# crowdbotp/socialways

Measured on AMD Instinct MI355X. Metric: GAN train steps/sec (256 scenes x 8 agents x 8+12 T per GPU step; fp32; social block on), higher is better.
Workload: dtype f32; 1 GPU; m1: 256 scenes x 8 agents x (8 obs + 12 pred) per GPU step = reference --batch-size 2048; use_social=True, n_unrolling_steps=1, info loss on; full=False, global_batch_scenes=256, parallelism=dp1, steps_per_graph_launch=32, settle_steps=992, rehearsal_regions=2, step_alg_bytes=5527040, inputs=z drawn on the host every step

## Files before the change

### socialways_amd/csrc/sw_wgrad.h

```cpp
#pragma once
#include <hip/hip_runtime.h>
#include <stddef.h>

#define SW_WG_MAXP 24
#define SW_WG_MAXSPLIT 256
#define SW_WG_WS_FLOATS ((size_t)SW_WG_MAXSPLIT * 65536)

struct WgProblem {
  const float* delta;
  const float* act;
  float* dW;
  float* db;
  float* db2;
  size_t ws_off;
  int ldd, lda, ldw, R, N, K, ones, accumulate;
  int nbn, nbk, nsplit, job0, out0;
  int pre;
  const float* act2;
  float* dW2;
  int lda2, ldw2, K2, row0;
};
struct WgBatch {
  int job0s[SW_WG_MAXP], out0s[SW_WG_MAXP];
  WgProblem p[SW_WG_MAXP];
  int np = 0, total_jobs = 0, total_out = 0;
  size_t top_reserved = 0;
};

struct WgAdam {
  float* w = nullptr;
  float* m = nullptr;
  float* v = nullptr;
  const float* g0 = nullptr;
  const float* step = nullptr;
  double lr = 0, beta1 = 0, beta2 = 0, eps = 0;
  size_t n = ~(size_t)0;
  const float* bc = nullptr;
  float* img = nullptr;
  const int* tab = nullptr;
};
__device__ __forceinline__ void wg_adam_bc_compute(const float* step, double beta1, double beta2, float& bc1, float& bc2s) {
  const float st = *step;
  bc1 = (float)(1 - pow(beta1, (double)st));
  bc2s = (float)sqrt(1 - pow(beta2, (double)st));
}
__device__ __forceinline__ void wg_adam_bc(const WgAdam& A, float& bc1, float& bc2s) {
  if (A.bc) {
    bc1 = A.bc[0];
    bc2s = A.bc[1];
    return;
  }
  wg_adam_bc_compute(A.step, A.beta1, A.beta2, bc1, bc2s);
}
struct WgAdamPre {
  size_t i;
  float m, v, w;
  int2 t;
};
__device__ __forceinline__ WgAdamPre wg_adam_pre(const WgAdam& A, const float* gptr) {
  WgAdamPre s;
  s.i = (size_t)(gptr - A.g0);
  s.t = int2{-1, -1};
  if (s.i >= A.n) {
    s.i = ~(size_t)0;
    s.m = s.v = s.w = 0.f;
    return s;
  }
  s.m = A.m[s.i];
  s.v = A.v[s.i];
  s.w = A.w[s.i];
  if (A.img) s.t = reinterpret_cast<const int2*>(A.tab)[s.i];
  return s;
}
__device__ __forceinline__ void wg_adam_fin(const WgAdam& A, const WgAdamPre& s, float bc1, float bc2s, float grad) {
  if (s.i == ~(size_t)0) return;
  const float m = (float)((double)s.m + (1 - A.beta1) * ((double)grad - (double)s.m));
  const float v = (float)(A.beta2 * s.v + (1 - A.beta2) * grad * grad);
  const float step_size = (float)(A.lr / bc1);
  const float denom = (float)((sqrtf(v) / bc2s) + A.eps);
  A.m[s.i] = m;
  A.v[s.i] = v;
  const float wn = s.w - step_size * m / denom;
  A.w[s.i] = wn;
  if (A.img) {
    if (s.t.x >= 0) A.img[s.t.x] = wn;
    if (s.t.y >= 0) A.img[s.t.y] = wn;
  }
}
__device__ __forceinline__ void wg_adam1(const WgAdam& A, float bc1, float bc2s, const float* gptr, float grad) {
  wg_adam_fin(A, wg_adam_pre(A, gptr), bc1, bc2s, grad);
}
int wg_reduce_launch_adam(WgBatch& b, float* ws, const WgAdam& ad, hipStream_t stream);
int wg_reduce_launch(WgBatch& b, float* ws, hipStream_t stream);
int wg_launch_adam(WgBatch& b, float* ws, WgAdam& ad, hipStream_t stream);

bool wg_shape_ok(int N, int K);
int wg_add(WgBatch& b, const float* delta, int ldd, const float* act, int lda, int R, int N, int K, float* dW,
           int ldw, float* db, float* db2, int accumulate);
int wg_add_tail(WgBatch& b, const float* delta, int ldd, const float* act, int lda, int R, int N, int K, float* dW,
                int ldw, const float* act2, int lda2, int K2, float* dW2, int ldw2, int row0, float* db, float* db2,
                int accumulate);
double wg_total_work(const WgBatch& b);
size_t wg_finalize(WgBatch& b);
int wg_launch(WgBatch& b, float* ws, hipStream_t stream);
int wg_add_pre(WgBatch& b, int N, int K, float* dW, int ldw, float* db, int nslices);
int wg_launch_finalized(WgBatch& b, float* ws, hipStream_t stream);
struct sw_wgrad_batch;
WgBatch* wg_pending(sw_wgrad_batch* h);
```

### socialways_amd/csrc/sw_wgrad.hip

```cpp
#include "../../include/socialways_hip.h"
#include "sw_common.h"
#include "sw_wgrad.h"
#include "sw_wgrad_dev.h"
#include <stdlib.h>

__host__ __device__ inline int wg_grid_jobs(int total_jobs) { return (total_jobs + 31) & ~31; }
#ifdef SW_WG_STAMP
__device__ unsigned long long g_wg_stamps[4 * 4096];
extern "C" int sw_debug_wg_stamps(unsigned long long* host, int n) {
  return hipMemcpyFromSymbol(host, HIP_SYMBOL(g_wg_stamps), sizeof(unsigned long long) * (size_t)n) == hipSuccess ? 0 : -1;
}
#endif
__global__ __launch_bounds__(SW_THREADS, 2) void wgrad_partial_kernel(WgBatch batch, float* __restrict__ ws,
                                                                      const float* __restrict__ adam_step, double beta1,
                                                                      double beta2, float* __restrict__ bc_out) {
  __shared__ __attribute__((aligned(16))) float red[SW_WG_RED_FLOATS];
  if ((int)blockIdx.x >= wg_grid_jobs(batch.total_jobs)) {
    if (threadIdx.x == 0) {
      float bc1, bc2s;
      wg_adam_bc_compute(adam_step, beta1, beta2, bc1, bc2s);
      bc_out[0] = bc1;
      bc_out[1] = bc2s;
    }
    return;
  }
  const int v = blockIdx.x, l = v >> 3;
  const int job = ((((l >> 2) << 3) + (v & 7)) << 2) + (l & 3);
  if (job >= batch.total_jobs) return;
#ifdef SW_WG_STAMP
  const unsigned long long t0 = wall_clock64();
#endif
  wg_job(batch, ws, job, red);
#ifdef SW_WG_STAMP
  if (threadIdx.x == 0 && blockIdx.x < 2048) {
    int p = 0;
    while (p + 1 < batch.np && job >= batch.job0s[p + 1]) ++p;
    unsigned long long* o = g_wg_stamps + (batch.total_jobs < 400 ? 4 * 2048 : 0) + 4 * blockIdx.x;
    o[0] = t0;
    o[1] = wall_clock64();
    o[2] = p;
    o[3] = batch.total_jobs;
  }
#endif
}
__device__ float g_wg_bc[2 * 64];
static float* wg_bc_slot() {
  static float* base[32] = {};
  static unsigned next = 0;
  int dev = -1;
  if (hipGetDevice(&dev) != hipSuccess || dev < 0 || dev >= 32) return nullptr;
  if (!base[dev]) {
    void* p = nullptr;
    if (hipGetSymbolAddress(&p, HIP_SYMBOL(g_wg_bc)) != hipSuccess) {
      (void)hipGetLastError();
      return nullptr;
    }
    base[dev] = (float*)p;
  }
  return base[dev] + 2 * (next++ % 64);
}

#ifndef SW_WG_RSUB
#define SW_WG_RSUB 4
#endif
#define SW_WG_REL (64 / SW_WG_RSUB)
__global__ __launch_bounds__(256) void wgrad_reduce_kernel(WgBatch batch, const float* __restrict__ ws, WgAdam ad) {
  const int gid = blockIdx.x * 256 + threadIdx.x;
  const int lane = gid & 63, el = lane % SW_WG_REL, sub = lane / SW_WG_REL;
  const int i = (gid >> 6) * SW_WG_REL + el;
  bool live = i < batch.total_out;
  int ii = live ? i : batch.total_out - 1;
  int p = 0;
#pragma unroll 1
  while (p + 1 < batch.np && ii >= batch.out0s[p + 1]) ++p;
  const WgProblem& P = batch.p[p];
  const int e = ii - P.out0;
  const int Kc = P.K + P.K2 + P.ones;
  const size_t stride = (size_t)P.N * Kc;
  const float* src = ws + P.ws_off + e;
  const int n = e / Kc, k = e - n * Kc;
  float* dst = k < P.K ? P.dW + (size_t)n * P.ldw + k : k < P.K + P.K2 ? P.dW2 + (size_t)n * P.ldw2 + (k - P.K) : P.db + n;
  float* dst2 = (k >= P.K + P.K2 && P.db2) ? P.db2 + n : nullptr;
  WgAdamPre a1 = {}, a2 = {};
  float old1 = 0.f, old2 = 0.f;
  if (ad.w) {
    a1 = wg_adam_pre(ad, dst);
    if (dst2) a2 = wg_adam_pre(ad, dst2);
  }
  if (P.accumulate) {
    old1 = *dst;
    if (dst2) old2 = *dst2;
  }
  float s = 0.f;
  float s1 = 0.f, s2 = 0.f, s3 = 0.f;
  int q = sub;
  for (; q + 3 * SW_WG_RSUB < P.nsplit; q += 4 * SW_WG_RSUB) {
    s += src[(size_t)q * stride];
    s1 += src[(size_t)(q + SW_WG_RSUB) * stride];
    s2 += src[(size_t)(q + 2 * SW_WG_RSUB) * stride];
    s3 += src[(size_t)(q + 3 * SW_WG_RSUB) * stride];
  }
  for (; q < P.nsplit; q += SW_WG_RSUB) s += src[(size_t)q * stride];
  s = (s + s1) + (s2 + s3);
#pragma unroll
  for (int o = SW_WG_REL; o < 64; o <<= 1) s += __shfl_xor(s, o);
  float bc1 = 1.f, bc2s = 1.f;
  if (ad.w) wg_adam_bc(ad, bc1, bc2s);
  if (!live || sub != 0) return;
  const float g = P.accumulate ? old1 + s : s;
  *dst = g;
  if (ad.w) wg_adam_fin(ad, a1, bc1, bc2s, g);
  if (dst2) {
    const float g2 = P.accumulate ? old2 + s : s;
    *dst2 = g2;
    if (ad.w) wg_adam_fin(ad, a2, bc1, bc2s, g2);
  }
}

bool wg_shape_ok(int N, int K) {
  for (int n0 = 0; n0 < N; n0 += 64)
    if (!wg_tiles(N - n0 < 64 ? N - n0 : 64, false)) return false;
  return K == 0 || wg_tiles(K, true) != 0;
}

static bool wg_span_ok(int R, int ld, int row0) {
  const long long rows = (long long)R / 4 + 4 + 8 * 4 * SW_WG_DEPTH + row0;
  return rows * ld * 4 < (1LL << 31);
}

int wg_add(WgBatch& b, const float* delta, int ldd, const float* act, int lda, int R, int N, int K, float* dW,
           int ldw, float* db, float* db2, int accumulate) {
  if (N > 256 || (ldd & 3) || (lda & 3)) return SW_ESHAPE;
  if (!wg_span_ok(R, ldd, 0) || !wg_span_ok(R, lda, 0)) return SW_ESHAPE;
  if (K < 1) return SW_ESHAPE;
  const int Nfull = N > 64 && (N & 63) && (N & 63) <= 32 && b.np + 2 * ((K + 63) / 64) <= SW_WG_MAXP ? (N & ~63) : N;
  for (int n0 = 0; n0 < N; n0 = (n0 == 0 ? Nfull : N)) {
    const int Nseg = n0 == 0 ? Nfull : N - Nfull;
    for (int c0 = 0; c0 < K; c0 += 64) {
      if (b.np >= SW_WG_MAXP) return SW_ESHAPE;
      const int c1 = c0 + 64 < K ? c0 + 64 : K;
      const bool has_ones = db && c1 == K;
      WgProblem& P = b.p[b.np++];
      P.delta = delta + n0; P.ldd = ldd; P.act = act + c0; P.lda = lda;
      P.R = R; P.N = Nseg; P.K = c1 - c0; P.ones = has_ones ? 1 : 0;
      P.dW = dW + (size_t)n0 * ldw + c0; P.ldw = ldw; P.db = has_ones ? db + n0 : nullptr;
      P.db2 = has_ones && db2 ? db2 + n0 : nullptr;
      P.accumulate = accumulate;
      P.pre = 0;
      P.act2 = nullptr; P.dW2 = nullptr; P.lda2 = P.ldw2 = P.K2 = P.row0 = 0;
      if (!wg_shape_ok(Nseg, P.K)) return SW_ESHAPE;
      P.nbn = (Nseg + 15) / 16;
      P.nbk = P.K > 0 ? wg_tiles(P.K, true) : 1;
    }
  }
  return SW_OK;
}

int wg_add_tail(WgBatch& b, const float* delta, int ldd, const float* act, int lda, int R, int N, int K, float* dW,
                int ldw, const float* act2, int lda2, int K2, float* dW2, int ldw2, int row0, float* db, float* db2,
                int accumulate) {
  if (N > 256 || (ldd & 3) || (lda & 3) || (lda2 & 3) || K != 64 || K2 != 4 || b.np >= SW_WG_MAXP)
    return SW_ESHAPE;
  if (row0 < 0 || !wg_span_ok(R, ldd, 0) || !wg_span_ok(R, lda, row0) || !wg_span_ok(R, lda2, 0)) return SW_ESHAPE;
  WgProblem& P = b.p[b.np++];
  P.delta = delta; P.ldd = ldd; P.act = act; P.lda = lda; P.R = R; P.N = N; P.K = K; P.ones = db ? 1 : 0;
  P.dW = dW; P.ldw = ldw; P.db = db; P.db2 = db ? db2 : nullptr; P.accumulate = accumulate; P.pre = 0;
  P.act2 = act2; P.lda2 = lda2; P.K2 = K2; P.dW2 = dW2; P.ldw2 = ldw2; P.row0 = row0;
  if (!wg_shape_ok(N, K)) return SW_ESHAPE;
  P.nbn = (N + 15) / 16;
  P.nbk = 4;
  return SW_OK;
}

int wg_add_pre(WgBatch& b, int N, int K, float* dW, int ldw, float* db, int nslices) {
  if (b.np >= SW_WG_MAXP || N < 1 || K < 1 || !db || nslices < 1) return SW_ESHAPE;
  WgProblem& P = b.p[b.np++];
  P.delta = nullptr; P.act = nullptr; P.ldd = P.lda = 0; P.R = 0;
  P.N = N; P.K = K; P.ones = 1; P.dW = dW; P.ldw = ldw; P.db = db; P.db2 = nullptr; P.accumulate = 0;
  P.nbn = (N + 15) / 16; P.nbk = (K + 1 + 15) / 16;
  P.act2 = nullptr; P.dW2 = nullptr; P.lda2 = P.ldw2 = P.K2 = P.row0 = 0;
  P.pre = nslices;
  b.top_reserved += (size_t)nslices * N * (K + 1);
  if (b.top_reserved > SW_WG_WS_FLOATS) return SW_ESHAPE;
  P.ws_off = SW_WG_WS_FLOATS - b.top_reserved;
  return SW_OK;
}

#ifndef SW_WG_GROUP_C0
#define SW_WG_GROUP_C0 256.0
#endif
#ifndef SW_WG_ROUND_UP
#define SW_WG_ROUND_UP 0.75
#endif
static double wg_cost(const WgProblem& P) {
  double c = 0;
  for (int n0 = 0; n0 < P.N; n0 += 64) {
    int ni = (P.N - n0 + 15) / 16;
    if (ni > 4) ni = 4;
    double per_group = ni * P.nbk * 32.0 + ni * (P.K2 + P.ones) * 4.0 + SW_WG_GROUP_C0;
    if (per_group < 192.0) per_group = 192.0;
    c += per_group;
  }
  return c * (P.R / 4.0 + 8.0);
}
double wg_total_work(const WgBatch& b) {
  double w = 0;
  for (int i = 0; i < b.np; ++i)
    if (!b.p[i].pre) w += wg_cost(b.p[i]);
  return w;
}

size_t wg_finalize(WgBatch& b) {
  {
    auto key = [](const WgProblem& P) { return P.pre ? 0 : (P.N + 63) / 64; };
    for (int i = 1; i < b.np; ++i) {
      const WgProblem t = b.p[i];
      int j = i;
      for (; j > 0 && key(b.p[j - 1]) < key(t); --j) b.p[j] = b.p[j - 1];
      b.p[j] = t;
    }
  }
  const double total = wg_total_work(b) + 1.0;
  static const double grain = 8192.0 * (1.0 + SW_WG_GROUP_C0 / 512.0);
  double target = total / grain / 4.0;
  if (target < 64.0) target = 64.0;
  const double maxwg = target >= 4096.0 ? 1024.0 : 512.0;
  if (target > maxwg) target = maxwg;
  const double small_env = 256.0;
  const bool one_per_cu = target > 256.0 && target < 448.0;
  if (one_per_cu) target = small_env;
  auto assign = [&](double tgt) {
    size_t ws = 0;
    int job = 0, out = 0;
    for (int i = 0; i < b.np; ++i) {
      WgProblem& P = b.p[i];
      const int NB = (P.N + 63) / 64;
      int ns;
      if (P.pre) {
        ns = P.pre;
      } else {
        const double share = tgt * wg_cost(P) / total / NB;
        ns = (int)(share + (share < 4.0 && maxwg <= 512.0 ? SW_WG_ROUND_UP : 0.5));
        int cap = (P.R + 127) / 128;
        if (ns > cap) ns = cap;
        if (ns > SW_WG_MAXSPLIT) ns = SW_WG_MAXSPLIT;
        if (ns < 1) ns = 1;
      }
      P.nsplit = ns;
      P.job0 = job;
      b.job0s[i] = job;
      b.out0s[i] = out;
      if (!P.pre) job += ns * NB;
      P.out0 = out;
      const int Kc = P.K + P.K2 + P.ones;
      out += P.N * Kc;
      if (!P.pre) {
        P.ws_off = ws;
        ws += (size_t)ns * P.N * Kc;
      }
    }
    b.total_jobs = job;
    b.total_out = out;
    return ws;
  };
  size_t ws = assign(target);
  const int limit = one_per_cu ? (int)small_env : (target >= maxwg ? (int)maxwg : 1 << 30);
  for (double tgt = target - 4.0; b.total_jobs > limit && tgt > 64.0; tgt -= 4.0) ws = assign(tgt);
  return ws + b.top_reserved;
}

struct sw_wgrad_batch {
  WgBatch b;
};
extern "C" sw_wgrad_batch* sw_wgrad_batch_new(void) { return new sw_wgrad_batch(); }
extern "C" void sw_wgrad_batch_free(sw_wgrad_batch* h) { delete h; }
WgBatch* wg_pending(sw_wgrad_batch* h) { return h ? &h->b : nullptr; }

int wg_launch(WgBatch& b, float* ws, hipStream_t stream) {
  if (b.np == 0) return SW_OK;
  size_t need = wg_finalize(b);
  if (need > SW_WG_WS_FLOATS) return SW_ESHAPE;
  return wg_launch_finalized(b, ws, stream);
}

int wg_reduce_launch_adam(WgBatch& b, float* ws, const WgAdam& ad, hipStream_t stream) {
  if (b.total_out == 0) return SW_OK;
  SW_LAUNCH(wgrad_reduce_kernel, dim3((b.total_out * SW_WG_RSUB + 255) / 256), dim3(256), 0, stream, b, ws, ad);
  SW_CHECK_LAUNCH("wgrad_reduce_kernel");
  return SW_OK;
}
int wg_reduce_launch(WgBatch& b, float* ws, hipStream_t stream) { return wg_reduce_launch_adam(b, ws, WgAdam(), stream); }
int wg_launch_adam(WgBatch& b, float* ws, WgAdam& ad, hipStream_t stream) {
  if (b.np == 0) return SW_OK;
  size_t need = wg_finalize(b);
  if (need > SW_WG_WS_FLOATS) return SW_ESHAPE;
  if (b.total_out == 0) return SW_OK;
  ad.bc = nullptr;
  if (b.total_jobs > 0) {
    float* bc = ad.w ? wg_bc_slot() : nullptr;
    SW_LAUNCH(wgrad_partial_kernel, dim3(wg_grid_jobs(b.total_jobs) + (bc ? 1 : 0)), dim3(SW_THREADS), 0, stream, b, ws, ad.step,
                       ad.beta1, ad.beta2, bc);
    SW_CHECK_LAUNCH("wgrad_partial_kernel");
    ad.bc = bc;
  }
  return wg_reduce_launch_adam(b, ws, ad, stream);
}

int wg_launch_finalized(WgBatch& b, float* ws, hipStream_t stream) {
  if (b.total_out == 0) return SW_OK;
  if (b.total_jobs > 0) {
    SW_LAUNCH(wgrad_partial_kernel, dim3(wg_grid_jobs(b.total_jobs)), dim3(SW_THREADS), 0, stream, b, ws, (const float*)nullptr,
                       0.0, 0.0, (float*)nullptr);
    SW_CHECK_LAUNCH("wgrad_partial_kernel");
  }
  return wg_reduce_launch(b, ws, stream);
}
```

### socialways_amd/csrc/sw_wgrad_dev.h

```cpp
#pragma once
#include <type_traits>
#include "sw_common.h"
#include "sw_wgrad.h"
#ifndef SW_WG_DEPTH
#define SW_WG_DEPTH 4
#endif
#ifndef SW_WG_DEPTH5
#define SW_WG_DEPTH5 2
#endif
#ifndef SW_WG_DEPTH_TAIL
#define SW_WG_DEPTH_TAIL SW_WG_DEPTH
#endif

#define SW_WG_RLD 69

typedef __amdgpu_buffer_rsrc_t wg_rsrc;
__device__ __forceinline__ wg_rsrc wg_make_rsrc(const float* base, unsigned bytes) {
  return __builtin_amdgcn_make_buffer_rsrc(const_cast<float*>(base), 0, (int)bytes, 0x00020000);
}
template <int NV>
__device__ __forceinline__ void wg_ldv(float (&v)[NV], wg_rsrc rs, unsigned off) {
  unsigned u[NV];
  if constexpr (NV == 4) {
    const auto q = __builtin_amdgcn_raw_buffer_load_b128(rs, (int)off, 0, 0);
    u[0] = q[0]; u[1] = q[1]; u[2] = q[2]; u[3] = q[3];
  } else if constexpr (NV == 3) {
    const auto q = __builtin_amdgcn_raw_buffer_load_b96(rs, (int)off, 0, 0);
    u[0] = q[0]; u[1] = q[1]; u[2] = q[2];
  } else if constexpr (NV == 2) {
    const auto q = __builtin_amdgcn_raw_buffer_load_b64(rs, (int)off, 0, 0);
    u[0] = q[0]; u[1] = q[1];
  } else {
    u[0] = __builtin_amdgcn_raw_buffer_load_b32(rs, (int)off, 0, 0);
  }
#pragma unroll
  for (int i = 0; i < NV; ++i) v[i] = __uint_as_float(u[i]);
}

__host__ __device__ inline int wg_tiles(int n, bool allow3) {
  if (n <= 16) return 1;
  for (int t = (n + 15) >> 4; t <= 4; ++t)
    if ((t != 3 || allow3) && n % t == 0) return t;
  return 0;
}

template <int NA, int KR, int K2, int ONES, int DSCALE = 1>
__device__ __forceinline__ void wg_run(const float* __restrict__ dbase, const float* __restrict__ abase, int ldd, int lda,
                                       int rbeg, int rend, int acol, int bcol, int lg, int ln,
                                       float* __restrict__ mine,
                                       const float* __restrict__ abase2, int lda2, int row0, int xoff) {
  constexpr int KT = KR, XC = K2 + ONES;
  f32x4 acc[NA][KT];
#pragma unroll
  for (int i = 0; i < NA; ++i) {
#pragma unroll
    for (int kt = 0; kt < KT; ++kt) acc[i][kt] = f32x4{0.f, 0.f, 0.f, 0.f};
  }
  float xacc[NA][XC > 0 ? XC : 1];
#pragma unroll
  for (int i = 0; i < NA; ++i) {
#pragma unroll
    for (int c = 0; c < (XC > 0 ? XC : 1); ++c) xacc[i][c] = 0.f;
  }
  constexpr int DEPTH = (K2 > 0 ? SW_WG_DEPTH_TAIL : SW_WG_DEPTH) * DSCALE;
  float a[DEPTH][NA], b[DEPTH][KT];
  f32x4 xq[DEPTH];
  const int abeg = K2 > 0 ? max(rbeg, row0) : rbeg, aend = max(abeg, rend);
  const wg_rsrc drs = wg_make_rsrc(dbase + (size_t)rbeg * ldd, (unsigned)(rend - rbeg) * (unsigned)ldd * 4u);
  const wg_rsrc ars = wg_make_rsrc(abase + (size_t)abeg * lda, (unsigned)(aend - abeg) * (unsigned)lda * 4u);
  const wg_rsrc xrs = wg_make_rsrc(abase2 + (size_t)rbeg * lda2, (unsigned)(rend - rbeg) * (unsigned)lda2 * 4u);
  unsigned doff = (unsigned)(lg * ldd + acol) * 4u, aoff = (unsigned)((rbeg - abeg + lg) * lda + bcol) * 4u;
  unsigned xoff2 = (unsigned)(lg * lda2) * 4u;
  const unsigned dstep = 16u * (unsigned)ldd, astep = 16u * (unsigned)lda, xstep = 16u * (unsigned)lda2;
  auto load = [&](float (&av)[NA], float (&bv)[KT], f32x4& xv) {
    wg_ldv<NA>(av, drs, doff);
    doff += dstep;
    wg_ldv<KR>(bv, ars, aoff);
    aoff += astep;
    if constexpr (K2 > 0) {
      float x4[4];
      wg_ldv<4>(x4, xrs, xoff2);
      xv = f32x4{x4[0], x4[1], x4[2], x4[3]};
      xoff2 += xstep;
    }
  };
#pragma unroll
  for (int q = 0; q < DEPTH - 1; ++q) load(a[q], b[q], xq[q]);
  for (int r = rbeg; r < rend; r += 4 * DEPTH) {
#pragma unroll
    for (int q = 0; q < DEPTH; ++q) {
      load(a[(q + DEPTH - 1) % DEPTH], b[(q + DEPTH - 1) % DEPTH], xq[(q + DEPTH - 1) % DEPTH]);
      asm volatile("" ::: "memory");
#pragma unroll
      for (int i = 0; i < NA; ++i) asm volatile("" : "+v"(a[q][i]));
#pragma unroll
      for (int kt = 0; kt < KT; ++kt) asm volatile("" : "+v"(b[q][kt]));
      if constexpr (K2 > 0) asm volatile("" : "+v"(xq[q]));
#pragma unroll
      for (int i = 0; i < NA; ++i) {
#pragma unroll
        for (int kt = 0; kt < KT; ++kt) {
          acc[i][kt] = SW_MFMA(a[q][i], b[q][kt], acc[i][kt]);
        }
      }
#pragma unroll
      for (int i = 0; i < NA; ++i) {
        if constexpr (K2 > 0) {
#pragma unroll
          for (int c = 0; c < K2; ++c) xacc[i][c] = fmaf(a[q][i], xq[q][c], xacc[i][c]);
        }
        if constexpr (ONES) xacc[i][K2] += a[q][i];
      }
    }
  }
#pragma unroll
  for (int i = 0; i < NA; ++i) {
#pragma unroll
    for (int kt = 0; kt < KT; ++kt) {
#pragma unroll
      for (int r = 0; r < 4; ++r) {
        const int orow = NA * (4 * lg + r) + i;
        if (KR * ln + kt < xoff) mine[orow * SW_WG_RLD + KR * ln + kt] = acc[i][kt][r];
      }
    }
  }
  if constexpr (XC > 0) {
#pragma unroll
    for (int i = 0; i < NA; ++i) {
#pragma unroll
      for (int c = 0; c < XC; ++c) {
        float v = xacc[i][c];
        v += __shfl_xor(v, 16);
        v += __shfl_xor(v, 32);
        if (lg == 0) mine[(NA * ln + i) * SW_WG_RLD + xoff + c] = v;
      }
    }
  }
}

#define SW_WG_RED_FLOATS (4 * 64 * SW_WG_RLD)
template <int DSCALE = 1>
__device__ __forceinline__ void wg_job(const WgBatch& batch, float* __restrict__ ws, int job, float* red) {
  const int lane = sw_lane(), wave = sw_wave(), ln = lane & 15, lg = lane >> 4;
  int p = 0;
#pragma unroll 1
  while (p + 1 < batch.np && job >= batch.job0s[p + 1]) ++p;
  const WgProblem& P = batch.p[p];
  const int j = job - P.job0;
  const int NB = (P.N + 63) >> 6;
  const int sg = j / NB, nb = j - sg * NB;
  const int s = sg * 4 + wave;
  const int N = P.N, K = P.K, Kc = P.K + P.K2 + P.ones;
  const int n0 = nb * 64;
  const int Nb = min(64, N - n0);
  const int NA = wg_tiles(Nb, false);
  const int KR = K > 0 ? wg_tiles(K, true) : 1;
  const int nsub = P.nsplit * 4;
  const int rows_per = (((P.R + nsub - 1) / nsub) + 3) & ~3;
  const int rbeg = __builtin_amdgcn_readfirstlane(min(P.R, s * rows_per));
  const int rend = __builtin_amdgcn_readfirstlane(min(P.R, rbeg + rows_per));
  const int acol = n0 + max(0, min(NA * ln, Nb - NA));
  const int bcol = max(0, min(KR * ln, K - KR));
  float* mine = red + wave * 64 * SW_WG_RLD;
#define WG_CASE(na, kr, k2, on)                                                                                     \
  case ((na * 8 + kr) * 2 + (k2 ? 1 : 0)) * 2 + on:                                                                 \
    wg_run<na, kr, k2, on, DSCALE>(P.delta, P.act, P.ldd, P.lda, rbeg, rend, acol, bcol, lg, ln,                      \
                                   mine, P.act2 ? P.act2 : P.delta, P.act2 ? P.lda2 : P.ldd, P.row0, K);            \
    break;
#define WG_CASES(na)                                                                                                \
  WG_CASE(na, 1, 0, 0) WG_CASE(na, 2, 0, 0) WG_CASE(na, 3, 0, 0) WG_CASE(na, 4, 0, 0)                               \
  WG_CASE(na, 1, 0, 1) WG_CASE(na, 2, 0, 1) WG_CASE(na, 3, 0, 1) WG_CASE(na, 4, 0, 1)                               \
  WG_CASE(na, 4, 4, 0) WG_CASE(na, 4, 4, 1)
  switch (((NA * 8 + KR) * 2 + (P.K2 ? 1 : 0)) * 2 + (P.ones ? 1 : 0)) {
    WG_CASES(1) WG_CASES(2) WG_CASES(4)
  }
#undef WG_CASES
#undef WG_CASE
  sw_barrier();
  float* out = ws + P.ws_off + (size_t)sg * N * Kc;
  const int rows = min(64, N - n0), cols = min(SW_WG_RLD, Kc);
  const int dq = SW_THREADS / cols, dr = SW_THREADS - dq * cols;
  int rr = threadIdx.x / cols, cc = threadIdx.x - rr * cols;
  const float* r0 = red, *r1 = red + 64 * SW_WG_RLD, *r2 = red + 2 * 64 * SW_WG_RLD, *r3 = red + 3 * 64 * SW_WG_RLD;
  for (int e = threadIdx.x; e < rows * cols; e += SW_THREADS) {
    const int o = rr * SW_WG_RLD + cc;
    const float v = (r0[o] + r1[o]) + (r2[o] + r3[o]);
    out[(size_t)(n0 + rr) * Kc + cc] = v;
    cc += dr;
    rr += dq;
    if (cc >= cols) {
      cc -= cols;
      ++rr;
    }
  }
}
```

Baseline: 2850 steps/s.

## Pad wgrad partial workspace to 16-byte rows and precompute per-problem dispatch metadata

Padding LDS reduction rows to 72 floats and workspace rows to a multiple of 4 lets the partial-sum epilogue and the accumulator stores use float4/float2 vector accesses. Per-problem values such as rows_per, the template case code, reciprocal multipliers for division and a padded leading dimension are now precomputed on the host. The kernels use a branchless unrolled key search with scalar-pinned metadata instead of a serial while loop, and the main K loop is peeled into whole groups plus a remainder. Together these cut integer division, scalar loads and scattered scalar LDS and global traffic, at the cost of extra workspace, a 16-byte alignment requirement on ws, and heavier register pressure.

```diff
diff --git a/socialways_amd/csrc/sw_wgrad.h b/socialways_amd/csrc/sw_wgrad.h
--- a/socialways_amd/csrc/sw_wgrad.h
+++ b/socialways_amd/csrc/sw_wgrad.h
@@ -9,23 +9,44 @@
 struct WgProblem {
   const float* delta;
   const float* act;
+  const float* act2;
+  size_t ws_off;
+  int ldd, lda, lda2, row0, R, N, K, job0;
+  int cases, rows_per, nbmul, ldp;
+  int K2, ones, nsplit, out0;
+  unsigned kcmul;
+  int ldw, ldw2, accumulate;
   float* dW;
+  float* dW2;
   float* db;
   float* db2;
-  size_t ws_off;
-  int ldd, lda, ldw, R, N, K, ones, accumulate;
-  int nbn, nbk, nsplit, job0, out0;
+  int nbk;
   int pre;
-  const float* act2;
-  float* dW2;
-  int lda2, ldw2, K2, row0;
 };
 struct WgBatch {
+  int total_jobs = 0, total_out = 0;
   int job0s[SW_WG_MAXP], out0s[SW_WG_MAXP];
   WgProblem p[SW_WG_MAXP];
-  int np = 0, total_jobs = 0, total_out = 0;
+  int np = 0;
   size_t top_reserved = 0;
 };
+
+#define WG_PIN(x) asm volatile("" ::"s"(x))
+__device__ __forceinline__ void wg_keys(const int (&keys)[SW_WG_MAXP], const int& total, int (&k)[SW_WG_MAXP], int& t) {
+  t = total;
+#pragma unroll
+  for (int i = 1; i < SW_WG_MAXP; ++i) k[i] = keys[i];
+  WG_PIN(t);
+#pragma unroll
+  for (int i = 1; i < SW_WG_MAXP; ++i) WG_PIN(k[i]);
+  k[0] = 0;
+}
+__device__ __forceinline__ int wg_find(const int (&k)[SW_WG_MAXP], int x) {
+  unsigned p = 0;
+#pragma unroll
+  for (int i = 1; i < SW_WG_MAXP; ++i) p += (unsigned)(k[i] - 1 - x) >> 31;
+  return (int)p;
+}
 
 struct WgAdam {
   float* w = nullptr;
diff --git a/socialways_amd/csrc/sw_wgrad.hip b/socialways_amd/csrc/sw_wgrad.hip
--- a/socialways_amd/csrc/sw_wgrad.hip
+++ b/socialways_amd/csrc/sw_wgrad.hip
@@ -2,11 +2,13 @@
 #include "sw_common.h"
 #include "sw_wgrad.h"
 #include "sw_wgrad_dev.h"
+#include <stdint.h>
 #include <stdlib.h>
 
 __host__ __device__ inline int wg_grid_jobs(int total_jobs) { return (total_jobs + 31) & ~31; }
 #ifdef SW_WG_STAMP
-__device__ unsigned long long g_wg_stamps[4 * 4096];
+#define SW_WG_STAMP_GEMM (2 * 2048 * 10)
+__device__ unsigned long long g_wg_stamps[SW_WG_STAMP_GEMM + 2 * 2048 * 6];
 extern "C" int sw_debug_wg_stamps(unsigned long long* host, int n) {
   return hipMemcpyFromSymbol(host, HIP_SYMBOL(g_wg_stamps), sizeof(unsigned long long) * (size_t)n) == hipSuccess ? 0 : -1;
 }
@@ -15,7 +17,9 @@
                                                                       const float* __restrict__ adam_step, double beta1,
                                                                       double beta2, float* __restrict__ bc_out) {
   __shared__ __attribute__((aligned(16))) float red[SW_WG_RED_FLOATS];
-  if ((int)blockIdx.x >= wg_grid_jobs(batch.total_jobs)) {
+  int keys[SW_WG_MAXP], total_jobs;
+  wg_keys(batch.job0s, batch.total_jobs, keys, total_jobs);
+  if ((int)blockIdx.x >= wg_grid_jobs(total_jobs)) {
     if (threadIdx.x == 0) {
       float bc1, bc2s;
       wg_adam_bc_compute(adam_step, beta1, beta2, bc1, bc2s);
@@ -26,21 +30,23 @@
   }
   const int v = blockIdx.x, l = v >> 3;
   const int job = ((((l >> 2) << 3) + (v & 7)) << 2) + (l & 3);
-  if (job >= batch.total_jobs) return;
+  if (job >= total_jobs) return;
 #ifdef SW_WG_STAMP
   const unsigned long long t0 = wall_clock64();
 #endif
-  wg_job(batch, ws, job, red);
-#ifdef SW_WG_STAMP
+#ifdef SW_WG_STAMP
+  unsigned long long mk[6] = {t0, t0, t0, t0, t0, t0};
+  wg_job(batch, keys, ws, job, red, mk);
   if (threadIdx.x == 0 && blockIdx.x < 2048) {
-    int p = 0;
-    while (p + 1 < batch.np && job >= batch.job0s[p + 1]) ++p;
-    unsigned long long* o = g_wg_stamps + (batch.total_jobs < 400 ? 4 * 2048 : 0) + 4 * blockIdx.x;
+    unsigned long long* o = g_wg_stamps + (batch.np <= 12 ? 10 * 2048 : 0) + 10 * blockIdx.x;
     o[0] = t0;
     o[1] = wall_clock64();
-    o[2] = p;
-    o[3] = batch.total_jobs;
-  }
+    o[2] = wg_find(keys, job);
+    o[3] = total_jobs;
+    for (int i = 0; i < 6; ++i) o[4 + i] = mk[i];
+  }
+#else
+  wg_job(batch, keys, ws, job, red);
 #endif
 }
 __device__ float g_wg_bc[2 * 64];
@@ -65,20 +71,38 @@
 #endif
 #define SW_WG_REL (64 / SW_WG_RSUB)
 __global__ __launch_bounds__(256) void wgrad_reduce_kernel(WgBatch batch, const float* __restrict__ ws, WgAdam ad) {
+#ifdef SW_WG_STAMP
+  const unsigned long long rt0 = wall_clock64();
+  unsigned long long rt1 = rt0, rt2 = rt0, rt3 = rt0;
+#endif
   const int gid = blockIdx.x * 256 + threadIdx.x;
-  const int lane = gid & 63, el = lane % SW_WG_REL, sub = lane / SW_WG_REL;
-  const int i = (gid >> 6) * SW_WG_REL + el;
-  bool live = i < batch.total_out;
-  int ii = live ? i : batch.total_out - 1;
-  int p = 0;
-#pragma unroll 1
-  while (p + 1 < batch.np && ii >= batch.out0s[p + 1]) ++p;
-  const WgProblem& P = batch.p[p];
-  const int e = ii - P.out0;
-  const int Kc = P.K + P.K2 + P.ones;
-  const size_t stride = (size_t)P.N * Kc;
-  const float* src = ws + P.ws_off + e;
-  const int n = e / Kc, k = e - n * Kc;
+  const int lane = threadIdx.x & 63, el = lane % SW_WG_REL, sub = lane / SW_WG_REL;
+  const int i0 = __builtin_amdgcn_readfirstlane((gid >> 6) * SW_WG_REL);
+  int keys[SW_WG_MAXP], total_out;
+  wg_keys(batch.out0s, batch.total_out, keys, total_out);
+  if (i0 >= total_out) return;
+  const int p = wg_find(keys, i0);
+  const WgProblem& Q = batch.p[p];
+  struct {
+    size_t ws_off;
+    int N, K, ldp, K2, ones, nsplit, out0;
+    unsigned kcmul;
+    int ldw, ldw2, accumulate;
+    float *dW, *dW2, *db, *db2;
+  } P = {Q.ws_off, Q.N, Q.K, Q.ldp, Q.K2, Q.ones, Q.nsplit, Q.out0, Q.kcmul, Q.ldw, Q.ldw2, Q.accumulate, Q.dW, Q.dW2, Q.db, Q.db2};
+  WG_PIN(P.ws_off); WG_PIN(P.N); WG_PIN(P.K); WG_PIN(P.ldp); WG_PIN(P.K2); WG_PIN(P.ones); WG_PIN(P.nsplit); WG_PIN(P.out0);
+  WG_PIN(P.kcmul); WG_PIN(P.ldw); WG_PIN(P.ldw2); WG_PIN(P.accumulate); WG_PIN(P.dW); WG_PIN(P.dW2); WG_PIN(P.db); WG_PIN(P.db2);
+  WG_PIN(ws); WG_PIN(ad.w); WG_PIN(ad.m); WG_PIN(ad.v); WG_PIN(ad.g0); WG_PIN(ad.n); WG_PIN(ad.img); WG_PIN(ad.tab);
+#ifdef SW_WG_STAMP
+  rt1 = wall_clock64();
+#endif
+  const int Kc = P.K + P.K2 + P.ones, nout = P.N * Kc;
+  const int ei = i0 - P.out0 + el;
+  const bool live = ei < nout;
+  const int e = live ? ei : nout - 1;
+  const int n = (int)__umulhi((unsigned)e << 1, P.kcmul), k = e - n * Kc;
+  const size_t stride = (size_t)P.N * P.ldp;
+  const float* src = ws + P.ws_off + (size_t)n * P.ldp + k;
   float* dst = k < P.K ? P.dW + (size_t)n * P.ldw + k : k < P.K + P.K2 ? P.dW2 + (size_t)n * P.ldw2 + (k - P.K) : P.db + n;
   float* dst2 = (k >= P.K + P.K2 && P.db2) ? P.db2 + n : nullptr;
   WgAdamPre a1 = {}, a2 = {};
@@ -91,6 +115,9 @@
     old1 = *dst;
     if (dst2) old2 = *dst2;
   }
+#ifdef SW_WG_STAMP
+  rt2 = wall_clock64();
+#endif
   float s = 0.f;
   float s1 = 0.f, s2 = 0.f, s3 = 0.f;
   int q = sub;
@@ -104,8 +131,18 @@
   s = (s + s1) + (s2 + s3);
 #pragma unroll
   for (int o = SW_WG_REL; o < 64; o <<= 1) s += __shfl_xor(s, o);
+#ifdef SW_WG_STAMP
+  asm volatile("" : "+v"(s));
+  rt3 = wall_clock64();
+#endif
   float bc1 = 1.f, bc2s = 1.f;
   if (ad.w) wg_adam_bc(ad, bc1, bc2s);
+#ifdef SW_WG_STAMP
+  if (threadIdx.x == 0 && blockIdx.x < 2048) {
+    unsigned long long* o = g_wg_stamps + SW_WG_STAMP_GEMM + (batch.np <= 12 ? 6 * 2048 : 0) + 6 * blockIdx.x;
+    o[0] = rt0; o[1] = rt1; o[2] = rt2; o[3] = rt3; o[4] = wall_clock64(); o[5] = p;
+  }
+#endif
   if (!live || sub != 0) return;
   const float g = P.accumulate ? old1 + s : s;
   *dst = g;
@@ -149,7 +186,6 @@
       P.pre = 0;
       P.act2 = nullptr; P.dW2 = nullptr; P.lda2 = P.ldw2 = P.K2 = P.row0 = 0;
       if (!wg_shape_ok(Nseg, P.K)) return SW_ESHAPE;
-      P.nbn = (Nseg + 15) / 16;
       P.nbk = P.K > 0 ? wg_tiles(P.K, true) : 1;
     }
   }
@@ -167,7 +203,6 @@
   P.dW = dW; P.ldw = ldw; P.db = db; P.db2 = db ? db2 : nullptr; P.accumulate = accumulate; P.pre = 0;
   P.act2 = act2; P.lda2 = lda2; P.K2 = K2; P.dW2 = dW2; P.ldw2 = ldw2; P.row0 = row0;
   if (!wg_shape_ok(N, K)) return SW_ESHAPE;
-  P.nbn = (N + 15) / 16;
   P.nbk = 4;
   return SW_OK;
 }
@@ -177,7 +212,7 @@
   WgProblem& P = b.p[b.np++];
   P.delta = nullptr; P.act = nullptr; P.ldd = P.lda = 0; P.R = 0;
   P.N = N; P.K = K; P.ones = 1; P.dW = dW; P.ldw = ldw; P.db = db; P.db2 = nullptr; P.accumulate = 0;
-  P.nbn = (N + 15) / 16; P.nbk = (K + 1 + 15) / 16;
+  P.nbk = (K + 1 + 15) / 16;
   P.act2 = nullptr; P.dW2 = nullptr; P.lda2 = P.ldw2 = P.K2 = P.row0 = 0;
   P.pre = nslices;
   b.top_reserved += (size_t)nslices * N * (K + 1);
@@ -253,12 +288,21 @@
       if (!P.pre) job += ns * NB;
       P.out0 = out;
       const int Kc = P.K + P.K2 + P.ones;
-      out += P.N * Kc;
+      out += (P.N * Kc + 15) & ~15;
+      const int nsub = ns * 4;
+      P.rows_per = (((P.R + nsub - 1) / nsub) + 3) & ~3;
+      P.nbmul = (65536 + NB - 1) / NB;
+      P.kcmul = (unsigned)(((1ULL << 31) + Kc - 1) / Kc);
+      P.ldp = P.pre ? Kc : (Kc + 3) & ~3;
+      const int Nl = P.N - 64 * (NB - 1);
+      const int kr = wg_tiles(P.K, true), tl = (P.K2 ? 2 : 0) + (P.ones ? 1 : 0);
+      P.cases = ((wg_tiles(64, false) * 8 + kr) * 4 + tl) | ((wg_tiles(Nl, false) * 8 + kr) * 4 + tl) << 8 | NB << 16;
       if (!P.pre) {
         P.ws_off = ws;
-        ws += (size_t)ns * P.N * Kc;
+        ws += (size_t)ns * P.N * P.ldp;
       }
     }
+    for (int i = b.np; i < SW_WG_MAXP; ++i) b.job0s[i] = b.out0s[i] = 0x7fffffff;
     b.total_jobs = job;
     b.total_out = out;
     return ws;
@@ -295,6 +339,7 @@
   size_t need = wg_finalize(b);
   if (need > SW_WG_WS_FLOATS) return SW_ESHAPE;
   if (b.total_out == 0) return SW_OK;
+  if ((uintptr_t)ws & 15) return SW_EARG;
   ad.bc = nullptr;
   if (b.total_jobs > 0) {
     float* bc = ad.w ? wg_bc_slot() : nullptr;
@@ -308,6 +353,7 @@
 
 int wg_launch_finalized(WgBatch& b, float* ws, hipStream_t stream) {
   if (b.total_out == 0) return SW_OK;
+  if ((uintptr_t)ws & 15) return SW_EARG;
   if (b.total_jobs > 0) {
     SW_LAUNCH(wgrad_partial_kernel, dim3(wg_grid_jobs(b.total_jobs)), dim3(SW_THREADS), 0, stream, b, ws, (const float*)nullptr,
                        0.0, 0.0, (float*)nullptr);
diff --git a/socialways_amd/csrc/sw_wgrad_dev.h b/socialways_amd/csrc/sw_wgrad_dev.h
--- a/socialways_amd/csrc/sw_wgrad_dev.h
+++ b/socialways_amd/csrc/sw_wgrad_dev.h
@@ -11,8 +11,23 @@
 #ifndef SW_WG_DEPTH_TAIL
 #define SW_WG_DEPTH_TAIL SW_WG_DEPTH
 #endif
-
-#define SW_WG_RLD 69
+#ifndef SW_WG_PEEL
+#define SW_WG_PEEL 1
+#endif
+
+#ifdef SW_WG_STAMP
+#define WG_MARKS_ARG , unsigned long long (&mk)[6]
+#define WG_MARKS_PASS , mk
+#define WG_MARK(i) mk[i] = wall_clock64()
+#else
+#define WG_MARKS_ARG
+#define WG_MARKS_PASS
+#define WG_MARK(i) ((void)0)
+#endif
+
+#define SW_WG_RLD 72
+static_assert(SW_WG_RLD % 4 == 0 && SW_WG_RLD >= 69, "16-byte LDS rows that hold 64 + 4 + 1 columns");
+static_assert(2 * 4 * 64 * SW_WG_RLD * 4 <= 160 * 1024, "two workgroups per CU must fit the 160 KB of LDS");
 
 typedef __amdgpu_buffer_rsrc_t wg_rsrc;
 __device__ __forceinline__ wg_rsrc wg_make_rsrc(const float* base, unsigned bytes) {
@@ -48,20 +63,8 @@
 __device__ __forceinline__ void wg_run(const float* __restrict__ dbase, const float* __restrict__ abase, int ldd, int lda,
                                        int rbeg, int rend, int acol, int bcol, int lg, int ln,
                                        float* __restrict__ mine,
-                                       const float* __restrict__ abase2, int lda2, int row0, int xoff) {
+                                       const float* __restrict__ abase2, int lda2, int row0, int xoff WG_MARKS_ARG) {
   constexpr int KT = KR, XC = K2 + ONES;
-  f32x4 acc[NA][KT];
-#pragma unroll
-  for (int i = 0; i < NA; ++i) {
-#pragma unroll
-    for (int kt = 0; kt < KT; ++kt) acc[i][kt] = f32x4{0.f, 0.f, 0.f, 0.f};
-  }
-  float xacc[NA][XC > 0 ? XC : 1];
-#pragma unroll
-  for (int i = 0; i < NA; ++i) {
-#pragma unroll
-    for (int c = 0; c < (XC > 0 ? XC : 1); ++c) xacc[i][c] = 0.f;
-  }
   constexpr int DEPTH = (K2 > 0 ? SW_WG_DEPTH_TAIL : SW_WG_DEPTH) * DSCALE;
   float a[DEPTH][NA], b[DEPTH][KT];
   f32x4 xq[DEPTH];
@@ -72,6 +75,7 @@
   unsigned doff = (unsigned)(lg * ldd + acol) * 4u, aoff = (unsigned)((rbeg - abeg + lg) * lda + bcol) * 4u;
   unsigned xoff2 = (unsigned)(lg * lda2) * 4u;
   const unsigned dstep = 16u * (unsigned)ldd, astep = 16u * (unsigned)lda, xstep = 16u * (unsigned)lda2;
+  WG_MARK(1);
   auto load = [&](float (&av)[NA], float (&bv)[KT], f32x4& xv) {
     wg_ldv<NA>(av, drs, doff);
     doff += dstep;
@@ -86,53 +90,105 @@
   };
 #pragma unroll
   for (int q = 0; q < DEPTH - 1; ++q) load(a[q], b[q], xq[q]);
+  asm volatile("" ::: "memory");
+  f32x4 acc[NA][KT];
+#pragma unroll
+  for (int i = 0; i < NA; ++i) {
+#pragma unroll
+    for (int kt = 0; kt < KT; ++kt) acc[i][kt] = f32x4{0.f, 0.f, 0.f, 0.f};
+  }
+  float xacc[NA][XC > 0 ? XC : 1];
+#pragma unroll
+  for (int i = 0; i < NA; ++i) {
+#pragma unroll
+    for (int c = 0; c < (XC > 0 ? XC : 1); ++c) xacc[i][c] = 0.f;
+  }
+  auto consume = [&](int q) {
+#pragma unroll
+    for (int i = 0; i < NA; ++i) asm volatile("" : "+v"(a[q][i]));
+#pragma unroll
+    for (int kt = 0; kt < KT; ++kt) asm volatile("" : "+v"(b[q][kt]));
+    if constexpr (K2 > 0) asm volatile("" : "+v"(xq[q]));
+#pragma unroll
+    for (int i = 0; i < NA; ++i) {
+#pragma unroll
+      for (int kt = 0; kt < KT; ++kt) {
+        acc[i][kt] = SW_MFMA(a[q][i], b[q][kt], acc[i][kt]);
+      }
+    }
+#pragma unroll
+    for (int i = 0; i < NA; ++i) {
+      if constexpr (K2 > 0) {
+#pragma unroll
+        for (int c = 0; c < K2; ++c) xacc[i][c] = fmaf(a[q][i], xq[q][c], xacc[i][c]);
+      }
+      if constexpr (ONES) xacc[i][K2] += a[q][i];
+    }
+  };
+#if SW_WG_PEEL
+  const int groups = (rend - rbeg + 3) >> 2, whole = groups / DEPTH, rest = groups - whole * DEPTH;
+  for (int t = 0; t < whole; ++t) {
+#else
   for (int r = rbeg; r < rend; r += 4 * DEPTH) {
+#endif
 #pragma unroll
     for (int q = 0; q < DEPTH; ++q) {
       load(a[(q + DEPTH - 1) % DEPTH], b[(q + DEPTH - 1) % DEPTH], xq[(q + DEPTH - 1) % DEPTH]);
       asm volatile("" ::: "memory");
-#pragma unroll
-      for (int i = 0; i < NA; ++i) asm volatile("" : "+v"(a[q][i]));
-#pragma unroll
-      for (int kt = 0; kt < KT; ++kt) asm volatile("" : "+v"(b[q][kt]));
-      if constexpr (K2 > 0) asm volatile("" : "+v"(xq[q]));
-#pragma unroll
-      for (int i = 0; i < NA; ++i) {
-#pragma unroll
-        for (int kt = 0; kt < KT; ++kt) {
-          acc[i][kt] = SW_MFMA(a[q][i], b[q][kt], acc[i][kt]);
+      consume(q);
+#ifdef SW_WG_STAMP
+#if SW_WG_PEEL
+      if (q == 0 && t == 0) WG_MARK(2);
+#else
+      if (q == 0 && r == rbeg) WG_MARK(2);
+#endif
+#endif
+    }
+  }
+#if SW_WG_PEEL
+#pragma unroll
+  for (int q = 0; q < DEPTH - 1; ++q) {
+    if (q < rest) consume(q);
+  }
+#endif
+  WG_MARK(3);
+#pragma unroll
+  for (int i = 0; i < NA; ++i) {
+#pragma unroll
+    for (int r = 0; r < 4; ++r) {
+      float* o = mine + (NA * (4 * lg + r) + i) * SW_WG_RLD + KR * ln;
+      if (KR * ln < xoff) {
+        if constexpr (KR == 4) {
+          *reinterpret_cast<float4*>(o) = float4{acc[i][0][r], acc[i][1][r], acc[i][2][r], acc[i][3][r]};
+        } else if constexpr (KR == 2) {
+          *reinterpret_cast<float2*>(o) = float2{acc[i][0][r], acc[i][1][r]};
+        } else {
+#pragma unroll
+          for (int kt = 0; kt < KT; ++kt) o[kt] = acc[i][kt][r];
         }
       }
-#pragma unroll
-      for (int i = 0; i < NA; ++i) {
-        if constexpr (K2 > 0) {
-#pragma unroll
-          for (int c = 0; c < K2; ++c) xacc[i][c] = fmaf(a[q][i], xq[q][c], xacc[i][c]);
-        }
-        if constexpr (ONES) xacc[i][K2] += a[q][i];
-      }
-    }
-  }
-#pragma unroll
-  for (int i = 0; i < NA; ++i) {
-#pragma unroll
-    for (int kt = 0; kt < KT; ++kt) {
-#pragma unroll
-      for (int r = 0; r < 4; ++r) {
-        const int orow = NA * (4 * lg + r) + i;
-        if (KR * ln + kt < xoff) mine[orow * SW_WG_RLD + KR * ln + kt] = acc[i][kt][r];
-      }
     }
   }
   if constexpr (XC > 0) {
 #pragma unroll
     for (int i = 0; i < NA; ++i) {
+      float xv[XC];
 #pragma unroll
       for (int c = 0; c < XC; ++c) {
         float v = xacc[i][c];
         v += __shfl_xor(v, 16);
         v += __shfl_xor(v, 32);
-        if (lg == 0) mine[(NA * ln + i) * SW_WG_RLD + xoff + c] = v;
+        xv[c] = v;
+      }
+      float* o = mine + (NA * ln + i) * SW_WG_RLD + xoff;
+      if (lg == 0) {
+        if constexpr (K2 == 4) {
+          *reinterpret_cast<float4*>(o) = float4{xv[0], xv[1], xv[2], xv[3]};
+          if constexpr (ONES) o[4] = xv[4];
+        } else {
+#pragma unroll
+          for (int c = 0; c < XC; ++c) o[c] = xv[c];
+        }
       }
     }
   }
@@ -140,23 +196,32 @@
 
 #define SW_WG_RED_FLOATS (4 * 64 * SW_WG_RLD)
 template <int DSCALE = 1>
-__device__ __forceinline__ void wg_job(const WgBatch& batch, float* __restrict__ ws, int job, float* red) {
+__device__ __forceinline__ void wg_job(const WgBatch& batch, const int (&keys)[SW_WG_MAXP], float* __restrict__ ws, int job,
+                                       float* red WG_MARKS_ARG) {
   const int lane = sw_lane(), wave = sw_wave(), ln = lane & 15, lg = lane >> 4;
-  int p = 0;
-#pragma unroll 1
-  while (p + 1 < batch.np && job >= batch.job0s[p + 1]) ++p;
-  const WgProblem& P = batch.p[p];
+  const int p = wg_find(keys, job);
+  const WgProblem& Q = batch.p[p];
+  struct {
+    const float *delta, *act, *act2;
+    size_t ws_off;
+    int ldd, lda, lda2, row0, R, N, K, job0, cases, rows_per, nbmul, ldp;
+  } P = {Q.delta, Q.act,  Q.act2, Q.ws_off, Q.ldd, Q.lda,   Q.lda2,     Q.row0,
+         Q.R,     Q.N,    Q.K,    Q.job0,   Q.cases, Q.rows_per, Q.nbmul, Q.ldp};
+  WG_PIN(P.delta); WG_PIN(P.act); WG_PIN(P.act2); WG_PIN(P.ws_off);
+  WG_PIN(P.ldd); WG_PIN(P.lda); WG_PIN(P.lda2); WG_PIN(P.row0); WG_PIN(P.R); WG_PIN(P.N); WG_PIN(P.K); WG_PIN(P.job0);
+  WG_PIN(P.cases); WG_PIN(P.rows_per); WG_PIN(P.nbmul); WG_PIN(P.ldp);
+  WG_MARK(0);
   const int j = job - P.job0;
-  const int NB = (P.N + 63) >> 6;
-  const int sg = j / NB, nb = j - sg * NB;
+  const int NB = P.cases >> 16;
+  const int sg = (int)(((unsigned)j * (unsigned)P.nbmul) >> 16), nb = j - sg * NB;
   const int s = sg * 4 + wave;
-  const int N = P.N, K = P.K, Kc = P.K + P.K2 + P.ones;
+  const int N = P.N, K = P.K;
   const int n0 = nb * 64;
   const int Nb = min(64, N - n0);
-  const int NA = wg_tiles(Nb, false);
-  const int KR = K > 0 ? wg_tiles(K, true) : 1;
-  const int nsub = P.nsplit * 4;
-  const int rows_per = (((P.R + nsub - 1) / nsub) + 3) & ~3;
+  const int cs = (nb == NB - 1 ? P.cases >> 8 : P.cases) & 255;
+  const int NA = cs >> 5;
+  const int KR = (cs >> 2) & 7;
+  const int rows_per = P.rows_per;
   const int rbeg = __builtin_amdgcn_readfirstlane(min(P.R, s * rows_per));
   const int rend = __builtin_amdgcn_readfirstlane(min(P.R, rbeg + rows_per));
   const int acol = n0 + max(0, min(NA * ln, Nb - NA));
@@ -165,32 +230,36 @@
 #define WG_CASE(na, kr, k2, on)                                                                                     \
   case ((na * 8 + kr) * 2 + (k2 ? 1 : 0)) * 2 + on:                                                                 \
     wg_run<na, kr, k2, on, DSCALE>(P.delta, P.act, P.ldd, P.lda, rbeg, rend, acol, bcol, lg, ln,                      \
-                                   mine, P.act2 ? P.act2 : P.delta, P.act2 ? P.lda2 : P.ldd, P.row0, K);            \
+                                   mine, P.act2 ? P.act2 : P.delta, P.act2 ? P.lda2 : P.ldd, P.row0, K WG_MARKS_PASS); \
     break;
 #define WG_CASES(na)                                                                                                \
   WG_CASE(na, 1, 0, 0) WG_CASE(na, 2, 0, 0) WG_CASE(na, 3, 0, 0) WG_CASE(na, 4, 0, 0)                               \
   WG_CASE(na, 1, 0, 1) WG_CASE(na, 2, 0, 1) WG_CASE(na, 3, 0, 1) WG_CASE(na, 4, 0, 1)                               \
   WG_CASE(na, 4, 4, 0) WG_CASE(na, 4, 4, 1)
-  switch (((NA * 8 + KR) * 2 + (P.K2 ? 1 : 0)) * 2 + (P.ones ? 1 : 0)) {
+  switch (cs) {
     WG_CASES(1) WG_CASES(2) WG_CASES(4)
   }
 #undef WG_CASES
 #undef WG_CASE
   sw_barrier();
-  float* out = ws + P.ws_off + (size_t)sg * N * Kc;
-  const int rows = min(64, N - n0), cols = min(SW_WG_RLD, Kc);
-  const int dq = SW_THREADS / cols, dr = SW_THREADS - dq * cols;
-  int rr = threadIdx.x / cols, cc = threadIdx.x - rr * cols;
-  const float* r0 = red, *r1 = red + 64 * SW_WG_RLD, *r2 = red + 2 * 64 * SW_WG_RLD, *r3 = red + 3 * 64 * SW_WG_RLD;
-  for (int e = threadIdx.x; e < rows * cols; e += SW_THREADS) {
-    const int o = rr * SW_WG_RLD + cc;
-    const float v = (r0[o] + r1[o]) + (r2[o] + r3[o]);
-    out[(size_t)(n0 + rr) * Kc + cc] = v;
-    cc += dr;
-    rr += dq;
-    if (cc >= cols) {
-      cc -= cols;
-      ++rr;
-    }
-  }
-}
+  const int ldp = P.ldp, c4 = ldp >> 2;
+  float* out = ws + P.ws_off + ((size_t)sg * N + n0) * ldp;
+  const float rc4 = __builtin_amdgcn_rcpf((float)c4);
+  const float4* r0 = reinterpret_cast<const float4*>(red);
+  constexpr int S4 = 64 * SW_WG_RLD / 4;
+  for (int c = threadIdx.x; c < Nb * c4; c += SW_THREADS) {
+    const int rr = (int)(((float)c + 0.5f) * rc4), cq = c - rr * c4;
+    const int o = rr * (SW_WG_RLD / 4) + cq;
+    const float4 v0 = r0[o], v1 = r0[o + S4], v2 = r0[o + 2 * S4], v3 = r0[o + 3 * S4];
+    float4 v;
+    v.x = (v0.x + v1.x) + (v2.x + v3.x);
+    v.y = (v0.y + v1.y) + (v2.y + v3.y);
+    v.z = (v0.z + v1.z) + (v2.z + v3.z);
+    v.w = (v0.w + v1.w) + (v2.w + v3.w);
+    reinterpret_cast<float4*>(out)[rr * c4 + cq] = v;
+#ifdef SW_WG_STAMP
+    if (c == (int)threadIdx.x) WG_MARK(4);
+#endif
+  }
+  WG_MARK(5);
+}
```

After: 2960 steps/s (median of 6 runs). +3.9%, better.
